# erhant/halo2-vectordb

Measured on AMD Instinct MI355X. Metric: constraints/sec, proving hot path (witness+layout+commit MSM+NTT), kmeans k=16 circuit, higher is better.
Workload: dtype u32x8 (BN254 Fr/Fq, 254-bit Montgomery)

## Files before the change

### halo2_vectordb_amd/csrc/limb9.hpp

```cpp
#pragma once
#include <math.h>

#include "field.hpp"

namespace vdb {

struct L9 {
  uint32_t l[9];
};
HD L9 l9_split(const u256& a) {
  L9 r;
#pragma unroll
  for (int k = 0; k < 9; k++) {
    int pb = 29 * k, wb = pb >> 5, ob = pb & 31;
    uint32_t lo = a.w[wb];
    uint32_t hi = wb + 1 < 8 ? a.w[wb + 1 < 8 ? wb + 1 : 0] : 0u;
    r.l[k] = ob ? ((lo >> ob) | (hi << (32 - ob))) : lo;
    if (k < 8) r.l[k] &= 0x1fffffffu;
  }
  return r;
}
HD L9 l9_split32(const u256& a) {
  L9 r;
  r.l[0] = (a.w[0] << 5) & 0x1fffffffu;
#pragma unroll
  for (int k = 1; k < 9; k++) {
    int pb = 29 * k - 5, wb = pb >> 5, ob = pb & 31;
    uint32_t lo = a.w[wb];
    uint32_t hi = wb + 1 < 8 ? a.w[wb + 1 < 8 ? wb + 1 : 0] : 0u;
    r.l[k] = ob ? ((lo >> ob) | (hi << (32 - ob))) : lo;
    if (k < 8) r.l[k] &= 0x1fffffffu;
  }
  return r;
}
HD u256 l9_pack(const L9& L) {
  u256 r;
  r.w[0] = L.l[0] | (L.l[1] << 29);
  r.w[1] = (L.l[1] >> 3) | (L.l[2] << 26);
  r.w[2] = (L.l[2] >> 6) | (L.l[3] << 23);
  r.w[3] = (L.l[3] >> 9) | (L.l[4] << 20);
  r.w[4] = (L.l[4] >> 12) | (L.l[5] << 17);
  r.w[5] = (L.l[5] >> 15) | (L.l[6] << 14);
  r.w[6] = (L.l[6] >> 18) | (L.l[7] << 11);
  r.w[7] = (L.l[7] >> 21) | (L.l[8] << 8);
  return r;
}
HD void l9_renorm(L9& x) {
  uint32_t c[8];
#pragma unroll
  for (int k = 0; k < 8; k++) c[k] = x.l[k] >> 29;
#pragma unroll
  for (int k = 0; k < 8; k++) x.l[k] &= 0x1fffffffu;
#pragma unroll
  for (int k = 1; k < 9; k++) x.l[k] += c[k - 1];
}
HD void l9_carry(L9& x) {
#pragma unroll
  for (int k = 0; k < 8; k++) {
    x.l[k + 1] += x.l[k] >> 29;
    x.l[k] &= 0x1fffffffu;
  }
}
HD L9 l9_add(const L9& a, const L9& b) {
  L9 r;
#pragma unroll
  for (int k = 0; k < 9; k++) r.l[k] = a.l[k] + b.l[k];
  return r;
}
HD L9 l9_sub(const L9& a, const L9& t, const uint32_t (&ckp)[9]) {
  L9 r;
#pragma unroll
  for (int k = 0; k < 9; k++) r.l[k] = a.l[k] + (ckp[k] - t.l[k]);
  return r;
}
HD L9 l9_neg(const L9& t, const uint32_t (&ckp)[9]) {
  L9 r;
#pragma unroll
  for (int k = 0; k < 9; k++) r.l[k] = ckp[k] - t.l[k];
  return r;
}
template <class M>
HD L9 l9_mul(const L9& a, const L9& b) {
  L9 r;
  mont_core29<M>(r.l, a.l, b.l);
  return r;
}
template <class M>
HD L9 l9_mul_shoup(const L9& v, const L9& w, const L9& wq) {
  L9 r;
  shoup_core29<M>(r.l, v.l, w.l, wq.l);
  return r;
}
template <class M>
HD L9 l9_mul2(const L9& a1, const L9& b1, const L9& a2, const L9& b2) {
  L9 r;
  mont_core29_2<M>(r.l, a1.l, b1.l, a2.l, b2.l);
  return r;
}
template <class M>
HD L9 l9_sqr(const L9& a) {
  L9 r;
  mont_sqr_core29<M>(r.l, a.l);
  return r;
}
template <class M>
HD u256 l9_canon(const L9& t) {
  return lazy_canon<M>(l9_pack(t));
}
template <class M>
HD bool l9_is_zero_mod(const L9& t) {
  uint32_t z = 0, e = 0;
#pragma unroll
  for (int k = 0; k < 9; k++) {
    z |= t.l[k];
    e |= t.l[k] ^ M::P29[k];
  }
  return z == 0 || e == 0;
}
template <class M>
inline double l9_offset_limbs(uint32_t K, uint32_t out[9]) {
  uint64_t carry = 0;
  for (int k = 0; k < 9; k++) {
    uint64_t v = (uint64_t)K * M::P29[k] + carry;
    out[k] = (uint32_t)(v & 0x1fffffffu);
    carry = v >> 29;
  }
  out[8] += (uint32_t)(carry << 29);
  out[0] += 1u << 29;
  for (int k = 1; k < 8; k++) out[k] += (1u << 29) - 1;
  out[8] -= 1;
  double cmax = 0;
  for (int k = 0; k < 8; k++) cmax = fmax(cmax, (double)out[k] / (double)(1u << 29));
  return cmax;
}

}
```

### halo2_vectordb_amd/csrc/ntt.hip

```cpp
#include <type_traits>
#include <vector>

#include "common.hpp"
#include "limb9.hpp"

namespace vdb {

#define NTT_THREADS 256
#define NTT_TILE 1024
#define NTT_MAX_PASSES 4
#define NTT_DEFAULT_COLGROUP 0x7fffffffu

struct NttPass {
  uint32_t log_n, S, log_inner, logG;
  uint32_t nprev;
  uint32_t prevS[NTT_MAX_PASSES];
  uint32_t first;
  uint32_t coset;
  uint32_t vslots;
  const u256* in_tab[4];
  uint32_t coset_out;
  uint32_t scale;
  uint32_t s0;
  uint64_t in_len;
  uint64_t in_stride, out_stride;
  uint32_t ren_mask;
  uint32_t ren_out;
  uint32_t blk0;
  const ColSrc* srcs;
  uint32_t n_blind;
  uint32_t n_cols;
  uint32_t col_group;
  u256 zeta1, zeta2, fin;
  u256 zeta0;
  uint32_t ckp[9];
  const uint32_t* sh_tab;
  uint32_t sh_res_log, sh_ns;
  int32_t sh_max_s;
};

__device__ __forceinline__ uint32_t bitrev_s(uint32_t x, uint32_t bits) { return bits ? (__brev(x) >> (32 - bits)) : 0u; }

__device__ __forceinline__ u256 l9_canon_wide(L9 x) {
  constexpr uint32_t MU = 2840127191u;
  const uint32_t q = __umulhi((x.l[8] + (x.l[7] >> 29)) << 3, MU) >> 24;
  uint64_t acc = 0;
#pragma unroll
  for (int k = 0; k < 9; k++) {
    const uint32_t nk = (k == 0 ? 0x20000000u : 0x1fffffffu) - FrParams::P29[k];
    acc += (uint64_t)x.l[k] + (uint64_t)q * nk;
    x.l[k] = (uint32_t)acc & 0x1fffffffu;
    acc >>= 29;
  }
  u256 v = l9_pack(x), t, p2, pp = mod_p<Fr>();
  u256_add(p2, pp, pp);
  uint32_t keep = u256_sub(t, v, p2);
#pragma unroll
  for (int i = 0; i < 8; i++) v.w[i] = keep ? v.w[i] : t.w[i];
  return lazy_canon<Fr>(v);
}
__device__ __forceinline__ L9 l9_mul(const L9& a, const L9& W) { return l9_mul<Fr>(a, W); }
__device__ __forceinline__ u256 l9_canon(const L9& t) { return l9_canon<Fr>(t); }

struct L9Planes {
  uint4* a;
  uint4* b;
  uint32_t* c;
};
__device__ __forceinline__ L9 lds_get(const L9Planes& P, uint32_t idx) {
  uint4 a = P.a[idx], b = P.b[idx];
  L9 r;
  r.l[0] = a.x; r.l[1] = a.y; r.l[2] = a.z; r.l[3] = a.w;
  r.l[4] = b.x; r.l[5] = b.y; r.l[6] = b.z; r.l[7] = b.w;
  r.l[8] = P.c[idx];
  return r;
}
__device__ __forceinline__ void lds_put(const L9Planes& P, uint32_t idx, const L9& v) {
  P.a[idx] = make_uint4(v.l[0], v.l[1], v.l[2], v.l[3]);
  P.b[idx] = make_uint4(v.l[4], v.l[5], v.l[6], v.l[7]);
  P.c[idx] = v.l[8];
}

template <uint32_t CS, uint32_t s, uint32_t step, class F>
__device__ __forceinline__ void ntt_static_steps(F&& f) {
  if constexpr (s < CS) {
    f(std::integral_constant<uint32_t, s>{}, std::integral_constant<uint32_t, step>{});
    ntt_static_steps<CS, (s + 1 < CS ? s + 2 : s + 1), step + 1>(f);
  }
}
constexpr uint32_t ntt_spec_sh_res_log(uint32_t cs) { return cs == 8 ? 0u : 2u; }
template <bool LAST, bool VS = false, uint32_t CS = 0, uint32_t CS0 = 0, uint32_t CREN = 0>
__global__ __launch_bounds__(NTT_THREADS) void k_ntt_pass(const u256* __restrict__ in, u256* __restrict__ out,
                                                         const u256* __restrict__ tw, const u256* __restrict__ tw_inter, NttPass p,
                                                         uint32_t tiles_per_col) {
  extern __shared__ uint4 smem[];
  constexpr bool SPEC = CS > 0;
  const uint32_t S = SPEC ? CS : p.S, P_logG = SPEC ? 10u - CS : p.logG, P_s0 = SPEC ? CS0 : p.s0, P_ren_mask = SPEC ? CREN : p.ren_mask;
  const uint32_t P_sh_res_log = SPEC ? ntt_spec_sh_res_log(CS) : p.sh_res_log, P_sh_ns = SPEC ? ((1u << (CS ? CS - 1 : 0)) >> ntt_spec_sh_res_log(CS)) : p.sh_ns;
  const int32_t P_sh_max_s = SPEC ? (int32_t)CS - 2 - (int32_t)ntt_spec_sh_res_log(CS) : p.sh_max_s;
  const bool P_shoup = SPEC ? true : p.sh_tab != nullptr, P_blk0 = SPEC ? true : p.blk0 != 0;
  const uint32_t m = 1u << S, G = 1u << P_logG, T = m * G;
  const uint32_t row = m + 1, NE = G * row, NW = m / 2 ? m / 2 : 1;
  L9Planes D, W;
  D.a = smem;
  D.b = D.a + NE;
  W.a = D.b + NE;
  W.b = W.a + NW;
  const uint32_t NS = P_shoup ? P_sh_ns : 0;
  L9Planes WS, WQ;
  WS.a = W.b + NW;
  WS.b = WS.a + NS;
  WQ.a = WS.b + NS;
  WQ.b = WQ.a + NS;
  D.c = reinterpret_cast<uint32_t*>(WQ.b + NS);
  W.c = D.c + NE;
  WS.c = W.c + NW;
  WQ.c = WS.c + NS;
  const uint32_t tid = threadIdx.x;
  uint32_t col, tile;
  if (p.col_group == 0) {
    col = blockIdx.x / tiles_per_col;
    tile = blockIdx.x % tiles_per_col;
  } else {
    const uint32_t per_group = p.col_group * tiles_per_col;
    const uint32_t grp = blockIdx.x / per_group, r = blockIdx.x % per_group;
    const uint32_t left = p.n_cols - grp * p.col_group, ncg = left < p.col_group ? left : p.col_group;
    col = grp * p.col_group + r % ncg;
    tile = r / ncg;
  }
  const u256* cin = in + (size_t)(VS ? col / p.vslots : col) * p.in_stride;
  const u256* ctab = nullptr;
  if constexpr (VS) {
    const uint32_t slot = col % p.vslots;
    ctab = slot == 0 ? p.in_tab[0] : (slot == 1 ? p.in_tab[1] : (slot == 2 ? p.in_tab[2] : p.in_tab[3]));
  }
  ColSrc csrc;
  const bool from_src = p.first && p.srcs != nullptr;
  if (from_src) csrc = p.srcs[col];
  u256* cout = out + (size_t)col * p.out_stride;

  uint64_t base;
  uint64_t jstride;
  uint64_t gstride;
  uint32_t i0 = 0, q0_base = 0, rdig = 0, rest = 1;
  if (!LAST) {
    uint32_t tiles_inner = (1u << p.log_inner) >> P_logG;
    uint32_t o = tile / tiles_inner;
    i0 = (tile % tiles_inner) << P_logG;
    base = ((uint64_t)o << (S + p.log_inner)) + i0;
    jstride = 1ull << p.log_inner;
    gstride = 1;
  } else {
    if (p.nprev == 0) {
      base = 0;
      jstride = 1;
      gstride = 0;
    } else {
      rest = 1u << (p.log_n - S - p.prevS[0]);
      q0_base = (tile / rest) << P_logG;
      rdig = tile % rest;
      base = ((uint64_t)q0_base * rest + rdig) << S;
      jstride = 1;
      gstride = (uint64_t)rest << S;
    }
  }

  for (uint32_t e = tid; e < m / 2; e += NTT_THREADS) lds_put(W, e, l9_split(ld256(tw + ((size_t)e << (p.log_n - S)))));
  for (uint32_t e = tid; e < NS; e += NTT_THREADS) {
    L9 ws, wq;
#pragma unroll
    for (int k = 0; k < 9; k++) {
      ws.l[k] = p.sh_tab[18 * e + k];
      wq.l[k] = p.sh_tab[18 * e + 9 + k];
    }
    lds_put(WS, e, ws);
    lds_put(WQ, e, wq);
  }
  const uint32_t mload = m >> P_s0, Tload = mload * G;
  L9 Z0, Z1, Z2;
  if (!VS && p.coset) {
    Z1 = l9_split(p.zeta1);
    Z2 = l9_split(p.zeta2);
    if (p.coset == 2) Z0 = l9_split(p.zeta0);
  }
  for (uint32_t e = tid; e < Tload; e += NTT_THREADS) {
    uint32_t j, g;
    if (!LAST) {
      g = e & (G - 1);
      j = e >> P_logG;
    } else {
      j = e & (mload - 1);
      g = e / mload;
    }
    uint64_t idx = base + j * jstride + g * gstride;
    L9 v;
    if (!p.first || idx < p.in_len) {
      v = l9_split(from_src ? colsrc_fetch(csrc, idx, 1ull << p.log_n, p.n_blind) : ld256(cin + idx));
      if constexpr (VS) {
        v = l9_mul(v, l9_split(ld256(ctab + idx)));
      } else if (p.coset) {
        uint32_t r3 = (uint32_t)(idx % 3);
        if (r3 == 1) v = l9_mul(v, Z1);
        else if (r3 == 2) v = l9_mul(v, Z2);
        else if (p.coset == 2) v = l9_mul(v, Z0);
      }
    } else {
#pragma unroll
      for (int k = 0; k < 9; k++) v.l[k] = 0;
    }
    for (uint32_t rep = 0; rep < (1u << P_s0); rep++) lds_put(D, g * row + j + rep * mload, v);
  }
  __syncthreads();
  auto do_step = [&](auto s_c, auto step_c) {
    const uint32_t s = s_c, step = step_c;
    const uint32_t logh = S - 1 - s, h = 1u << logh;
    const bool ren = (P_ren_mask >> step) & 1;
    if (s + 1 < S) {
      const uint32_t h2 = h >> 1, lh1 = logh ? logh - 1 : 0;
      auto radix4 = [&](auto first_c, auto ren_c, auto shoup_c, auto s2_c) {
        constexpr bool FIRST = decltype(first_c)::value, REN = decltype(ren_c)::value, SHOUP = decltype(shoup_c)::value, S2 = decltype(s2_c)::value;
        for (uint32_t t = tid; t < T / 4; t += NTT_THREADS) {
          uint32_t g, r, blk;
          if (S2) {
            const uint32_t lb = P_logG + lh1;
            blk = ((t >> lb) + blockIdx.x + (blockIdx.x >> 8)) & 3u;
            g = (t >> lh1) & (G - 1);
            r = t & (h2 - 1);
          } else {
            const uint32_t gi = t & ((m >> 2) - 1);
            g = t >> (S - 2);
            r = gi & (h2 - 1);
            blk = gi >> lh1;
          }
          const uint32_t j0 = g * row + (blk << (logh + 1)) + r;
          L9 x0 = lds_get(D, j0), x1 = lds_get(D, j0 + h2), x2 = lds_get(D, j0 + h), x3 = lds_get(D, j0 + h + h2);
          if (REN) {
            l9_renorm(x0);
            l9_renorm(x1);
            l9_renorm(x2);
            l9_renorm(x3);
          }
          if (FIRST) {
            L9 a0 = l9_add(x0, x2), a2 = l9_sub(x0, x2, p.ckp);
            L9 a1 = l9_add(x1, x3), a3 = l9_sub(x1, x3, p.ckp);
            l9_carry(a1);
            const L9 t3 = l9_mul(a3, lds_get(W, m >> 2));
            x0 = l9_add(a0, a1);
            x1 = l9_sub(a0, a1, p.ckp);
            x2 = l9_add(a2, t3);
            x3 = l9_sub(a2, t3, p.ckp);
          } else if (S2 && blk == 0) {
            l9_carry(x2);
            l9_carry(x3);
            L9 a0 = l9_add(x0, x2), a2 = l9_sub(x0, x2, p.ckp);
            L9 a1 = l9_add(x1, x3), a3 = l9_sub(x1, x3, p.ckp);
            l9_carry(a1);
            L9 t3;
            if (SHOUP) {
              const uint32_t iq = (m >> 2) >> P_sh_res_log;
              t3 = l9_mul_shoup<Fr>(a3, lds_get(WS, iq), lds_get(WQ, iq));
            } else {
              t3 = l9_mul(a3, lds_get(W, m >> 2));
            }
            x0 = l9_add(a0, a1);
            x1 = l9_sub(a0, a1, p.ckp);
            x2 = l9_add(a2, t3);
            x3 = l9_sub(a2, t3, p.ckp);
          } else if (SHOUP) {
            const uint32_t e = bitrev_s(blk, s) << logh, rl = P_sh_res_log;
            const uint32_t i0 = e >> rl, i1 = (e >> 1) >> rl, i2 = ((e >> 1) + (m >> 2)) >> rl;
            const L9 ws = lds_get(WS, i0), wq = lds_get(WQ, i0);
            const L9 t2 = l9_mul_shoup<Fr>(x2, ws, wq), t3 = l9_mul_shoup<Fr>(x3, ws, wq);
            const L9 a0 = l9_add(x0, t2), a2 = l9_sub(x0, t2, p.ckp);
            const L9 a1 = l9_add(x1, t3), a3 = l9_sub(x1, t3, p.ckp);
            const L9 u1 = l9_mul_shoup<Fr>(a1, lds_get(WS, i1), lds_get(WQ, i1));
            const L9 u3 = l9_mul_shoup<Fr>(a3, lds_get(WS, i2), lds_get(WQ, i2));
            x0 = l9_add(a0, u1);
            x1 = l9_sub(a0, u1, p.ckp);
            x2 = l9_add(a2, u3);
            x3 = l9_sub(a2, u3, p.ckp);
          } else {
            const uint32_t e = bitrev_s(blk, s) << logh;
            const L9 w = lds_get(W, e);
            const L9 t2 = l9_mul(x2, w), t3 = l9_mul(x3, w);
            const L9 a0 = l9_add(x0, t2), a2 = l9_sub(x0, t2, p.ckp);
            const L9 a1 = l9_add(x1, t3), a3 = l9_sub(x1, t3, p.ckp);
            const L9 u1 = l9_mul(a1, lds_get(W, e >> 1));
            const L9 u3 = l9_mul(a3, lds_get(W, (e >> 1) + (m >> 2)));
            x0 = l9_add(a0, u1);
            x1 = l9_sub(a0, u1, p.ckp);
            x2 = l9_add(a2, u3);
            x3 = l9_sub(a2, u3, p.ckp);
          }
          lds_put(D, j0, x0);
          lds_put(D, j0 + h2, x1);
          lds_put(D, j0 + h, x2);
          lds_put(D, j0 + h + h2, x3);
        }
      };
      using T_ = std::true_type;
      using F_ = std::false_type;
      const bool s2 = s == 2 && !ren && P_blk0;
      if (s == 0) {
        if (ren) radix4(T_{}, T_{}, F_{}, F_{});
        else radix4(T_{}, F_{}, F_{}, F_{});
      } else if (P_shoup && (int32_t)s <= P_sh_max_s) {
        if (ren) radix4(F_{}, T_{}, T_{}, F_{});
        else if (s2) radix4(F_{}, F_{}, T_{}, T_{});
        else radix4(F_{}, F_{}, T_{}, F_{});
      } else {
        if (ren) radix4(F_{}, T_{}, F_{}, F_{});
        else if (s2) radix4(F_{}, F_{}, F_{}, T_{});
        else radix4(F_{}, F_{}, F_{}, F_{});
      }
    } else {
      for (uint32_t b = tid; b < T / 2; b += NTT_THREADS) {
        const uint32_t g = b >> (S - 1), pj = b & ((m >> 1) - 1);
        const uint32_t r = pj & (h - 1), blk = pj >> logh, j0 = (blk << (logh + 1)) + r;
        const uint32_t a0 = g * row + j0, a1 = a0 + h;
        L9 u = lds_get(D, a0), v = lds_get(D, a1);
        if (ren) {
          l9_renorm(u);
          l9_renorm(v);
        }
        if (s) v = l9_mul(v, lds_get(W, bitrev_s(blk, s) << logh));
        lds_put(D, a0, l9_add(u, v));
        lds_put(D, a1, l9_sub(u, v, p.ckp));
      }
    }
    __syncthreads();
  };
  if constexpr (SPEC) {
    ntt_static_steps<CS, CS0, 0>(do_step);
  } else {
    uint32_t step = 0;
    for (uint32_t s = P_s0; s < S; step++) {
      do_step(s, step);
      s += (s + 1 < S) ? 2 : 1;
    }
  }
  L9 FIN, ZO1, ZO2;
  if (LAST && p.scale) FIN = l9_split(p.fin);
  if (LAST && p.coset_out) {
    ZO1 = l9_split(p.zeta2);
    ZO2 = l9_split(p.zeta1);
  }
  constexpr uint32_t EPT = NTT_TILE / NTT_THREADS;
  u256 twv[EPT];
  if (!LAST) {
#pragma unroll
    for (uint32_t it = 0; it < EPT; it++) {
      const uint32_t e = tid + it * NTT_THREADS;
      const uint32_t g = e & (G - 1), q = e >> P_logG;
      const uint64_t ex = ((uint64_t)q * ((uint64_t)i0 + g)) << (p.log_n - S - p.log_inner);
      if (e < T) twv[it] = ld256(tw_inter + ex);
    }
  }
#pragma unroll
  for (uint32_t it = 0; it < EPT; it++) {
    const uint32_t e = tid + it * NTT_THREADS;
    if (e >= T) break;
    uint32_t g = e & (G - 1), q = e >> P_logG;
    L9 v = lds_get(D, g * row + bitrev_s(q, S));
    if (p.ren_out) l9_renorm(v);
    if (!LAST) {
      v = l9_mul(v, l9_split(twv[it]));
      st256(cout + base + (uint64_t)q * jstride + g, l9_pack(v));
    } else {
      uint64_t pos;
      if (p.nprev == 0) {
        pos = q;
      } else {
        pos = (uint64_t)q0_base + g;
        uint32_t r = rdig;
        uint32_t shift = 0;
        for (uint32_t l = 0; l < p.nprev; l++) shift += p.prevS[l];
        for (int l = (int)p.nprev - 1; l >= 1; l--) {
          shift -= p.prevS[l];
          uint32_t ql = r & ((1u << p.prevS[l]) - 1);
          r >>= p.prevS[l];
          pos += (uint64_t)ql << shift;
        }
        pos += (uint64_t)q << (p.log_n - S);
      }
      if (p.scale) {
        v = l9_mul(v, FIN);
        const uint32_t r3 = p.coset_out ? (uint32_t)(pos % 3) : 0u;
        if (r3) v = l9_mul(v, r3 == 1 ? ZO1 : ZO2);
        st256(cout + pos, l9_canon(v));
      } else {
        const uint32_t r3 = p.coset_out ? (uint32_t)(pos % 3) : 0u;
        st256(cout + pos, r3 ? l9_canon(l9_mul(v, r3 == 1 ? ZO1 : ZO2)) : l9_canon_wide(v));
      }
    }
  }
}

__global__ __launch_bounds__(256) void k_twiddles(u256* __restrict__ tw, u256 omega, u256 m32, uint64_t n, uint32_t chunk) {
  uint64_t t = (uint64_t)blockIdx.x * blockDim.x + threadIdx.x;
  uint64_t lo = t * chunk;
  if (lo >= n) return;
  u256 w = mont_pow<Fr>(omega, u256_from_u64(lo));
  for (uint32_t i = 0; i < chunk && lo + i < n; i++) {
    st256(tw + lo + i, fr_mul(w, m32));
    w = fr_mul(w, omega);
  }
}

static const u256* get_twiddles(uint32_t log_n, const u256& omega, const u256& factor, bool scaled, int* err) {
  Context& c = ctx();
  Context::TwKey key{log_n | (scaled ? 0x80000000u : 0u), omega};
  auto it = c.twiddles.find(key);
  if (it != c.twiddles.end()) return it->second;
  uint64_t n = 1ull << log_n;
  u256* tw = nullptr;
  hipError_t e = hipMalloc(&tw, n * sizeof(u256));
  if (e != hipSuccess) {
    *err = hip_fail(e, "hipMalloc(twiddles)", __FILE__, __LINE__);
    return nullptr;
  }
  uint32_t chunk = 16;
  uint64_t threads = (n + chunk - 1) / chunk;
  {
    VDB_PROF("k_twiddles");
    hipLaunchKernelGGL(k_twiddles, dim3((unsigned)((threads + 255) / 256)), dim3(256), 0, c.stream, tw, omega, factor, n, chunk);
  }
  e = hipGetLastError();
  if (e != hipSuccess) {
    *err = hip_fail(e, "k_twiddles", __FILE__, __LINE__);
    (void)hipFree(tw);
    return nullptr;
  }
  c.twiddles[key] = tw;
  return tw;
}

static void limbs29(const u256& a, uint32_t extra_top , uint32_t out[9]) {
  for (int k = 0; k < 9; k++) {
    const int bit = 29 * k, wd = bit >> 5, sh = bit & 31;
    uint64_t v = wd < 8 ? (uint64_t)a.w[wd] >> sh : 0;
    if (sh && wd + 1 < 8) v |= (uint64_t)a.w[wd + 1] << (32 - sh);
    if (wd + 1 == 8 && sh) v |= (uint64_t)extra_top << (32 - sh);
    if (wd == 8) v = extra_top >> sh;
    out[k] = (uint32_t)v & 0x1fffffffu;
  }
}
static const uint32_t* get_shoup_table(uint32_t log_n, const u256& omega, uint32_t S, uint32_t res_log, int* err) {
  Context& c = ctx();
  Context::TwKey key{log_n | (S << 8) | (res_log << 16) | 0x40000000u, omega};
  auto it = c.twiddles.find(key);
  if (it != c.twiddles.end()) return reinterpret_cast<const uint32_t*>(it->second);
  const uint32_t m = 1u << S, ns = (m / 2) >> res_log;
  std::vector<uint32_t> tab((size_t)ns * 18);
  const u256 p = mod_p<Fr>();
  const u256 step = mont_pow<Fr>(omega, u256_from_u64(((uint64_t)1 << (log_n - S)) << res_log));
  u256 cur = mont_one<Fr>();
  for (uint32_t j = 0; j < ns; j++) {
    const u256 w = from_mont<Fr>(cur);
    limbs29(w, 0, &tab[18 * (size_t)j]);
    u256 r = w;
    uint32_t q[9] = {0, 0, 0, 0, 0, 0, 0, 0, 0};
    for (int b = 260; b >= 0; b--) {
      u256 d;
      u256_add(d, r, r);
      u256 t;
      const uint32_t borrow = u256_sub(t, d, p);
      r = borrow ? d : t;
      if (!borrow) q[b / 29] |= 1u << (b % 29);
    }
    for (int k = 0; k < 9; k++) tab[18 * (size_t)j + 9 + k] = q[k];
    cur = fr_mul(cur, step);
  }
  uint32_t* d = nullptr;
  hipError_t e = hipMalloc(&d, tab.size() * sizeof(uint32_t));
  if (e != hipSuccess) {
    *err = hip_fail(e, "hipMalloc(shoup table)", __FILE__, __LINE__);
    return nullptr;
  }
  e = hipMemcpy(d, tab.data(), tab.size() * sizeof(uint32_t), hipMemcpyHostToDevice);
  if (e != hipSuccess) {
    *err = hip_fail(e, "hipMemcpy(shoup table)", __FILE__, __LINE__);
    (void)hipFree(d);
    return nullptr;
  }
  c.twiddles[key] = reinterpret_cast<u256*>(d);
  return d;
}

int ntt_dev(u256* data, u256* out_or_null, size_t n_cols, uint32_t log_n, const u256& omega, bool scale_ninv,
            bool coset_in, size_t in_len, const ColSrc* srcs, uint32_t n_blind, bool coset_out, const u256* in_scale, const u256* const* in_tabs,
            uint32_t vslots) {
  Context& c = ctx();
  if (n_cols == 0) return VDB_OK;
  if (log_n > 26) {
    set_error("ntt: log_n > 26 unsupported");
    return VDB_ERR_ARG;
  }
  const uint64_t n = 1ull << log_n;
  const uint64_t in_stride = in_len ? in_len : n;
  if (!in_len) in_len = n;
  u256* dst = out_or_null ? out_or_null : data;
  if (!out_or_null && in_stride != n) {
    set_error("ntt: in-place transform needs in_len == n");
    return VDB_ERR_ARG;
  }
  if (vslots && (!out_or_null || !in_tabs || vslots > 4 || srcs || coset_in || n_cols % vslots)) {
    set_error("ntt: virtual columns need an output buffer and their input tables");
    return VDB_ERR_ARG;
  }
  if (srcs && (!out_or_null || in_len != n || log_n <= 10)) {
    set_error("ntt: column sources need an output buffer and a multi-pass size");
    return VDB_ERR_ARG;
  }
  int err = VDB_OK;
  const u256 m32 = host_fr_from_u64(32);
  const u256* tw = get_twiddles(log_n, omega, m32, false, &err);
  if (!tw) return err;

  uint32_t L, S[NTT_MAX_PASSES];
  if (log_n <= 10) {
    L = 1;
    S[0] = log_n;
  } else {
    static const uint32_t max_s = getenv("VDB_NTT_MAX_S") ? (uint32_t)atoi(getenv("VDB_NTT_MAX_S")) : 9u;
    uint32_t ms = max_s >= 4 && max_s <= 9 ? max_s : 9u;
    while ((log_n + ms - 1) / ms > NTT_MAX_PASSES) ms++;
    L = (log_n + ms - 1) / ms;
    for (uint32_t l = 0; l < L; l++) S[l] = log_n / L + (l < log_n % L ? 1 : 0);
  }
  const u256 fin = scale_ninv ? fr_mul(mont_inv<Fr>(host_fr_from_u64(n)), m32) : m32;
  const u256* tw_scaled = tw;
  if (scale_ninv && L > 1) {
    tw_scaled = get_twiddles(log_n, omega, fin, true, &err);
    if (!tw_scaled) return err;
  }
  u256 z1 = host_zeta(), z2 = fr_mul(z1, z1);
  z1 = fr_mul(z1, m32);
  z2 = fr_mul(z2, m32);
  u256 z0 = m32;
  if (in_scale) {
    z0 = fr_mul(z0, *in_scale);
    z1 = fr_mul(z1, *in_scale);
    z2 = fr_mul(z2, *in_scale);
  }
  static const bool shoup_on = !(getenv("VDB_NTT_SHOUP") && getenv("VDB_NTT_SHOUP")[0] == '0');
  uint32_t ckp[9];
  const double cmax = l9_offset_limbs<FrParams>(14, ckp);

  size_t chunk_cols = n_cols;
  u256* scratch = nullptr;
  if (L > 1) {
    size_t max_cols = ((size_t)2 << 30) / (n * sizeof(u256));
    if (max_cols < 1) max_cols = 1;
    if (chunk_cols > max_cols) chunk_cols = max_cols;
    if (vslots) chunk_cols = chunk_cols / vslots * vslots ? chunk_cols / vslots * vslots : vslots;
    scratch = (u256*)scratch_get(3, chunk_cols * n * sizeof(u256));
    if (!scratch) return VDB_ERR_OOM;
  }
  static const uint32_t col_group = getenv("VDB_NTT_COLGROUP") ? (uint32_t)strtoul(getenv("VDB_NTT_COLGROUP"), nullptr, 10) : NTT_DEFAULT_COLGROUP;
  for (size_t c0 = 0; c0 < n_cols; c0 += chunk_cols) {
    size_t nc = n_cols - c0 < chunk_cols ? n_cols - c0 : chunk_cols;
    uint32_t done_bits = 0;
    for (uint32_t l = 0; l < L; l++) {
      NttPass p;
      memset(&p, 0, sizeof(p));
      p.log_n = log_n;
      p.S = S[l];
      p.log_inner = log_n - done_bits - S[l];
      p.first = (l == 0);
      const bool last = (l == L - 1);
      p.coset = (l == 0 && coset_in) ? (in_scale ? 2u : 1u) : ((l == 0 && vslots) ? 3u : 0u);
      p.vslots = vslots;
      for (uint32_t t = 0; t < vslots; t++) p.in_tab[t] = in_tabs[t];
      p.zeta0 = z0;
      p.in_len = in_len;
      p.srcs = (l == 0 && srcs) ? srcs + c0 : nullptr;
      p.n_blind = n_blind;
      p.n_cols = (uint32_t)nc;
      p.col_group = last ? 0u : (col_group < nc ? col_group : (uint32_t)nc);
      p.zeta1 = z1;
      p.zeta2 = z2;
      p.fin = fin;
      memcpy(p.ckp, ckp, sizeof(ckp));
      p.scale = last && scale_ninv && L == 1;
      p.coset_out = last && coset_out;
      p.s0 = (l == 0 && !last && S[0] >= 3 && in_len * 4 <= n) ? 2 : 0;
      {
        double b = 1.0001;
        uint32_t step = 0;
        for (uint32_t st = p.s0; st < S[l]; step++) {
          if (st + 1 < S[l]) {
            if (st == 0) {
              b = 1.0 + 2.0 * cmax;
            } else {
              if (b + cmax >= 6.1 || b + 2.0 * cmax >= 7.95) {
                p.ren_mask |= 1u << step;
                b = 1.0001;
              }
              b += 2.0 * cmax;
            }
            st += 2;
          } else {
            if (st == 0) {
              b = 1.0 + cmax;
            } else {
              if (b >= 6.1 || b + cmax >= 7.95) {
                p.ren_mask |= 1u << step;
                b = 1.0001;
              }
              b += cmax;
            }
            st += 1;
          }
        }
        const bool out_mul = !last || p.scale || p.coset_out;
        static const bool blk0_on = !(getenv("VDB_NTT_BLK0") && getenv("VDB_NTT_BLK0")[0] == '0');
        p.blk0 = blk0_on ? 1u : 0u;
        static const bool always = getenv("VDB_NTT_REN_OUT") && getenv("VDB_NTT_REN_OUT")[0] == '1';
        p.ren_out = (always || (out_mul && b >= 6.1)) ? 1u : 0u;
      }
      const u256* src;
      u256* out;
      if (l == 0) {
        src = srcs ? scratch : data + (vslots ? c0 / vslots : c0) * in_stride;
        p.in_stride = in_stride;
      } else {
        src = scratch;
        p.in_stride = n;
      }
      if (last) {
        out = dst + c0 * n;
        p.out_stride = n;
      } else {
        out = scratch;
        p.out_stride = n;
      }
      uint32_t m = 1u << S[l];
      if (L == 1) {
        p.logG = 0;
        p.nprev = 0;
      } else {
        p.logG = 10 - S[l];
        const uint32_t room = last ? S[0] : p.log_inner;
        if (p.logG > room) p.logG = room;
        p.nprev = l;
        for (uint32_t q = 0; q < l && q < NTT_MAX_PASSES; q++) p.prevS[q] = S[q];
      }
      uint32_t G = 1u << p.logG;
      uint32_t tiles = (uint32_t)(n / ((uint64_t)m * G));
      size_t lds = (size_t)(G * (m + 1) + (m / 2 ? m / 2 : 1)) * (2 * sizeof(uint4) + sizeof(uint32_t));
      p.sh_tab = nullptr;
      p.sh_res_log = p.sh_ns = 0;
      p.sh_max_s = -1;
      if (shoup_on && S[l] >= 4) {
        const size_t room = (160 * 1024) / 3;
        uint32_t rl = 0;
        while (rl + 2 < S[l] && lds + (size_t)((m / 2) >> rl) * 72 > room) rl++;
        const int32_t max_s = (int32_t)S[l] - 2 - (int32_t)rl;
        if (lds + (size_t)((m / 2) >> rl) * 72 <= room && max_s >= 1) {
          p.sh_tab = get_shoup_table(log_n, omega, S[l], rl, &err);
          if (!p.sh_tab) return err;
          p.sh_res_log = rl;
          p.sh_ns = (m / 2) >> rl;
          p.sh_max_s = max_s;
          lds += (size_t)p.sh_ns * 72;
        }
      }
      dim3 grid((unsigned)(nc * tiles));
      if (lds > 64 * 1024) {
        bool& raised = c.ntt_lds_raised;
        if (!raised) {
          VDB_HIP(hipFuncSetAttribute((const void*)k_ntt_pass<true>, hipFuncAttributeMaxDynamicSharedMemorySize, 96 * 1024));
          VDB_HIP(hipFuncSetAttribute((const void*)k_ntt_pass<false>, hipFuncAttributeMaxDynamicSharedMemorySize, 96 * 1024));
          VDB_HIP(hipFuncSetAttribute((const void*)k_ntt_pass<true, true>, hipFuncAttributeMaxDynamicSharedMemorySize, 96 * 1024));
          VDB_HIP(hipFuncSetAttribute((const void*)k_ntt_pass<false, true>, hipFuncAttributeMaxDynamicSharedMemorySize, 96 * 1024));
          raised = true;
        }
      }
      static const bool spec_on = !(getenv("VDB_NTT_SPEC") && getenv("VDB_NTT_SPEC")[0] == '0');
      const u256* twi = last ? tw : (l == 0 ? tw_scaled : tw);
      const bool vs = (l == 0 && vslots);
      auto spec = [&](uint32_t cs, uint32_t cs0, uint32_t cren) {
        const uint32_t rl = ntt_spec_sh_res_log(cs);
        return spec_on && L > 1 && p.S == cs && p.s0 == cs0 && p.ren_mask == cren && p.logG == 10 - cs && p.sh_tab && p.blk0 && p.sh_res_log == rl &&
               p.sh_ns == ((1u << (cs - 1)) >> rl) && p.sh_max_s == (int32_t)cs - 2 - (int32_t)rl;
      };
#define NTT_LAUNCH(...) hipLaunchKernelGGL((k_ntt_pass<__VA_ARGS__>), grid, dim3(NTT_THREADS), lds, c.stream, src, out, tw, twi, p, tiles)
      {
        VDB_PROF("k_ntt_pass");
        if (last) {
          if (vs) NTT_LAUNCH(true, true);
          else if (spec(8, 0, 4)) NTT_LAUNCH(true, false, 8, 0, 4);
          else if (spec(9, 0, 20)) NTT_LAUNCH(true, false, 9, 0, 20);
          else NTT_LAUNCH(true, false);
        } else {
          if (vs && spec(8, 0, 4)) NTT_LAUNCH(false, true, 8, 0, 4);
          else if (vs) NTT_LAUNCH(false, true);
          else if (spec(8, 0, 4)) NTT_LAUNCH(false, false, 8, 0, 4);
          else if (spec(9, 2, 4)) NTT_LAUNCH(false, false, 9, 2, 4);
          else if (spec(9, 0, 20)) NTT_LAUNCH(false, false, 9, 0, 20);
          else NTT_LAUNCH(false, false);
        }
      }
#undef NTT_LAUNCH
      VDB_LAUNCH_CHECK();
      done_bits += S[l];
    }
  }
  return VDB_OK;
}

struct CosetMix {
  const u256* tab[4];
  u256 c[4][4];
};
__global__ __launch_bounds__(256) void k_cosets_combine(const u256* __restrict__ P, uint64_t n, uint32_t n_slots, CosetMix mx, u256* __restrict__ out) {
  const uint64_t i = (uint64_t)blockIdx.x * blockDim.x + threadIdx.x;
  if (i >= n) return;
  u256 v[4];
#pragma unroll
  for (uint32_t t = 0; t < 4; t++)
    if (t < n_slots) v[t] = fr_mul(ld256(P + t * n + i), ld256(mx.tab[t] + i));
#pragma unroll
  for (uint32_t j = 0; j < 4; j++) {
    if (j >= n_slots) break;
    u256 acc = fr_mul(v[0], mx.c[j][0]);
#pragma unroll
    for (uint32_t t = 1; t < 4; t++)
      if (t < n_slots) acc = fr_add(acc, fr_mul(v[t], mx.c[j][t]));
    st256(out + j * n + i, acc);
  }
}

u256 host_coset_shift(uint32_t k, uint32_t t) {
  static const uint32_t rev[4] = {0, 2, 1, 3};
  return fr_mul(host_zeta(), mont_pow<Fr>(host_root_of_unity(k + 2), u256_from_u64(rev[t & 3])));
}

static int host_cols_roundtrip(vdb_fr* const* cols, size_t n_cols, size_t n, u256** dbuf, bool upload) {
  Context& c = ctx();
  size_t bytes = n * sizeof(u256);
  if (upload) {
    *dbuf = (u256*)scratch_get(0, n_cols * bytes);
    if (!*dbuf) return VDB_ERR_OOM;
    for (size_t i = 0; i < n_cols; i++) VDB_HIP(hipMemcpyAsync(*dbuf + i * n, cols[i], bytes, hipMemcpyHostToDevice, c.stream));
  } else {
    for (size_t i = 0; i < n_cols; i++) VDB_HIP(hipMemcpyAsync(cols[i], *dbuf + i * n, bytes, hipMemcpyDeviceToHost, c.stream));
    VDB_HIP(hipStreamSynchronize(c.stream));
  }
  return VDB_OK;
}

}

using namespace vdb;

extern "C" {

int vdb_ntt_batch_dev(vdb_fr* cols_dev, size_t n_cols, uint32_t log_n, const vdb_fr* omega, int flags) {
  VDB_REQUIRE_INIT();
  VDB_ARG(cols_dev && omega, "null pointer");
  u256 w;
  memcpy(&w, omega, 32);
  return ntt_dev(as_u256(cols_dev), nullptr, n_cols, log_n, w, (flags & VDB_NTT_INVERSE_SCALE) != 0, false, 0, nullptr, 0, false, nullptr);
}
int vdb_ntt_batch(vdb_fr* const* cols, size_t n_cols, uint32_t log_n, const vdb_fr* omega, int flags) {
  VDB_REQUIRE_INIT();
  VDB_ARG(cols && omega, "null pointer");
  if (n_cols == 0) return VDB_OK;
  u256* d = nullptr;
  int rc = host_cols_roundtrip(cols, n_cols, (size_t)1 << log_n, &d, true);
  if (rc) return rc;
  rc = vdb_ntt_batch_dev(reinterpret_cast<vdb_fr*>(d), n_cols, log_n, omega, flags);
  if (rc) return rc;
  return host_cols_roundtrip(cols, n_cols, (size_t)1 << log_n, &d, false);
}
int vdb_lagrange_to_coeff_dev(vdb_fr* cols_dev, size_t n_cols, uint32_t k) {
  VDB_REQUIRE_INIT();
  VDB_ARG(cols_dev && k <= 26, "bad argument");
  u256 w = mont_inv<Fr>(host_root_of_unity(k));
  return ntt_dev(as_u256(cols_dev), nullptr, n_cols, k, w, true, false, 0, nullptr, 0, false, nullptr);
}
int vdb_lagrange_to_coeff_src_dev(const vdb_colsrc* src_dev, vdb_fr* coeff_dev, size_t n_cols, uint32_t k, uint32_t n_blind) {
  VDB_REQUIRE_INIT();
  VDB_ARG(src_dev && coeff_dev && k <= 26 && k > 10, "bad argument (column sources are supported for k > 10)");
  u256 w = mont_inv<Fr>(host_root_of_unity(k));
  return ntt_dev(nullptr, as_u256(coeff_dev), n_cols, k, w, true, false, 0, reinterpret_cast<const ColSrc*>(src_dev), n_blind, false, nullptr);
}
int vdb_lagrange_to_coeff(vdb_fr* const* cols, size_t n_cols, uint32_t k) {
  VDB_REQUIRE_INIT();
  VDB_ARG(cols, "null pointer");
  if (n_cols == 0) return VDB_OK;
  u256* d = nullptr;
  int rc = host_cols_roundtrip(cols, n_cols, (size_t)1 << k, &d, true);
  if (rc) return rc;
  rc = vdb_lagrange_to_coeff_dev(reinterpret_cast<vdb_fr*>(d), n_cols, k);
  if (rc) return rc;
  return host_cols_roundtrip(cols, n_cols, (size_t)1 << k, &d, false);
}
int vdb_coeff_to_extended_dev(const vdb_fr* coeff_dev, vdb_fr* ext_dev, size_t n_cols, uint32_t k, uint32_t ext_k) {
  VDB_REQUIRE_INIT();
  VDB_ARG(coeff_dev && ext_dev && k + ext_k <= 26, "bad argument");
  u256 w = host_root_of_unity(k + ext_k);
  return ntt_dev(const_cast<u256*>(as_u256(coeff_dev)), as_u256(ext_dev), n_cols, k + ext_k, w, false, true, (size_t)1 << k, nullptr, 0, false, nullptr);
}
int vdb_coeff_to_extended_scaled_dev(const vdb_fr* coeff_dev, vdb_fr* ext_dev, size_t n_cols, uint32_t k, uint32_t ext_k, const vdb_fr* scale) {
  VDB_REQUIRE_INIT();
  VDB_ARG(coeff_dev && ext_dev && scale && k + ext_k <= 26, "bad argument");
  u256 w = host_root_of_unity(k + ext_k), sv;
  memcpy(&sv, scale, 32);
  return ntt_dev(const_cast<u256*>(as_u256(coeff_dev)), as_u256(ext_dev), n_cols, k + ext_k, w, false, true, (size_t)1 << k, nullptr, 0, false, &sv);
}
int vdb_extended_to_coeff_dev(vdb_fr* ext_dev, size_t n_cols, uint32_t k, uint32_t ext_k) {
  VDB_REQUIRE_INIT();
  VDB_ARG(ext_dev && k + ext_k <= 26, "bad argument");
  u256 w = mont_inv<Fr>(host_root_of_unity(k + ext_k));
  return ntt_dev(as_u256(ext_dev), nullptr, n_cols, k + ext_k, w, true, false, 0, nullptr, 0, true, nullptr);
}
int vdb_coeff_to_cosets_dev(const vdb_fr* coeff_dev, vdb_fr* cosets_dev, size_t n_cols, uint32_t k, uint32_t n_slots, const vdb_fr* scale_or_null) {
  VDB_REQUIRE_INIT();
  VDB_ARG(coeff_dev && cosets_dev && k + 2 <= 26 && n_slots >= 1 && n_slots <= 4, "bad argument");
  if (n_cols == 0) return VDB_OK;
  Context& c = ctx();
  const uint64_t n = 1ull << k;
  const u256 m32 = host_fr_from_u64(32);
  const u256* tabs[4] = {nullptr, nullptr, nullptr, nullptr};
  int err = VDB_OK;
  if (scale_or_null) {
    u256 sv;
    memcpy(&sv, scale_or_null, 32);
    u256* buf = (u256*)scratch_get(6, (size_t)n_slots * n * sizeof(u256));
    if (!buf) return VDB_ERR_OOM;
    const uint32_t chunk = 16;
    const uint64_t threads = (n + chunk - 1) / chunk;
    for (uint32_t t = 0; t < n_slots; t++) {
      hipLaunchKernelGGL(k_twiddles, dim3((unsigned)((threads + 255) / 256)), dim3(256), 0, c.stream, buf + t * n, host_coset_shift(k, t), fr_mul(m32, sv), n, chunk);
      tabs[t] = buf + t * n;
    }
    VDB_LAUNCH_CHECK();
  } else {
    for (uint32_t t = 0; t < n_slots; t++) {
      tabs[t] = get_twiddles(k, host_coset_shift(k, t), m32, false, &err);
      if (!tabs[t]) return err;
    }
  }
  return ntt_dev(const_cast<u256*>(as_u256(coeff_dev)), as_u256(cosets_dev), n_cols * n_slots, k, host_root_of_unity(k), false, false, 0, nullptr, 0, false, nullptr,
                 tabs, n_slots);
}
int vdb_cosets_to_coeff_dev(vdb_fr* cosets_dev, vdb_fr* coeff_dev, uint32_t k, uint32_t n_slots) {
  VDB_REQUIRE_INIT();
  VDB_ARG(cosets_dev && coeff_dev && k + 2 <= 26 && n_slots >= 1 && n_slots <= 4, "bad argument");
  Context& c = ctx();
  const uint64_t n = 1ull << k;
// ... 56 lines not shown
```

Before: 1.892 billion.

## Use Shoup precomputed multipliers for all twiddle products in specialized NTT passes

In the specialized 256- and 512-point NTT kernels, every remaining Montgomery twiddle multiplication is replaced with a Shoup multiply. This covers the radix-4 inner constant, the radix-2 stage twiddle, the coset zeta scaling and the inter-pass twiddle. The shared-memory twiddle table is dropped, and device-side per-element Shoup records (value plus quotient, 80 bytes each) are built once and cached for the inter-pass multiply. The aim is cheaper field multiplies and less LDS use, paid for with more than double the global-memory bytes for inter-pass twiddle loads and extra cached table memory. Host-side Shoup table generation is factored into a shared header.

```diff
diff --git a/halo2_vectordb_amd/csrc/limb9.hpp b/halo2_vectordb_amd/csrc/limb9.hpp
--- a/halo2_vectordb_amd/csrc/limb9.hpp
+++ b/halo2_vectordb_amd/csrc/limb9.hpp
@@ -91,6 +91,32 @@
   shoup_core29<M>(r.l, v.l, w.l, wq.l);
   return r;
 }
+HD void limbs29(const u256& a, uint32_t out[9]) {
+#pragma unroll
+  for (int k = 0; k < 9; k++) {
+    const int bit = 29 * k, wd = bit >> 5, sh = bit & 31;
+    uint64_t v = (uint64_t)a.w[wd] >> sh;
+    if (sh && wd + 1 < 8) v |= (uint64_t)a.w[wd + 1 < 8 ? wd + 1 : 0] << (32 - sh);
+    out[k] = (uint32_t)v & 0x1fffffffu;
+  }
+}
+HD void shoup_pair29(const u256& w, uint32_t out[18]) {
+  limbs29(w, out);
+  const u256 p = mod_p<Fr>();
+  u256 r = w;
+#pragma unroll
+  for (int k = 8; k >= 0; k--) {
+    uint32_t d = 0;
+    for (int j = 28; j >= 0; j--) {
+      u256 s, t;
+      u256_add(s, r, r);
+      const uint32_t borrow = u256_sub(t, s, p);
+      r = borrow ? s : t;
+      d |= (borrow ^ 1u) << j;
+    }
+    out[9 + k] = d;
+  }
+}
 template <class M>
 HD L9 l9_mul2(const L9& a1, const L9& b1, const L9& a2, const L9& b2) {
   L9 r;
diff --git a/halo2_vectordb_amd/csrc/ntt.hip b/halo2_vectordb_amd/csrc/ntt.hip
--- a/halo2_vectordb_amd/csrc/ntt.hip
+++ b/halo2_vectordb_amd/csrc/ntt.hip
@@ -3,6 +3,7 @@
 
 #include "common.hpp"
 #include "limb9.hpp"
+#include "shoup_tables.hpp"
 
 namespace vdb {
 
@@ -37,9 +38,33 @@
   const uint32_t* sh_tab;
   uint32_t sh_res_log, sh_ns;
   int32_t sh_max_s;
+  const uint32_t* sh2_tab;
+  const uint4* tw_rec;
+  uint32_t zsh[3][18];
 };
 
 __device__ __forceinline__ uint32_t bitrev_s(uint32_t x, uint32_t bits) { return bits ? (__brev(x) >> (32 - bits)) : 0u; }
+__device__ __forceinline__ L9 kconst(const uint32_t* k) {
+  L9 r;
+#pragma unroll
+  for (int i = 0; i < 9; i++) r.l[i] = k[i];
+  return r;
+}
+__device__ __forceinline__ void ld_pair18(const uint32_t* e, L9& w, L9& wq) {
+  const uint2* q = reinterpret_cast<const uint2*>(e);
+  uint32_t t[18];
+#pragma unroll
+  for (int i = 0; i < 9; i++) {
+    const uint2 v = q[i];
+    t[2 * i] = v.x;
+    t[2 * i + 1] = v.y;
+  }
+#pragma unroll
+  for (int i = 0; i < 9; i++) {
+    w.l[i] = t[i];
+    wq.l[i] = t[9 + i];
+  }
+}
 
 __device__ __forceinline__ u256 l9_canon_wide(L9 x) {
   constexpr uint32_t MU = 2840127191u;
@@ -88,19 +113,20 @@
     ntt_static_steps<CS, (s + 1 < CS ? s + 2 : s + 1), step + 1>(f);
   }
 }
-constexpr uint32_t ntt_spec_sh_res_log(uint32_t cs) { return cs == 8 ? 0u : 2u; }
-template <bool LAST, bool VS = false, uint32_t CS = 0, uint32_t CS0 = 0, uint32_t CREN = 0>
+constexpr uint32_t ntt_spec_sh_res_log(uint32_t cs, bool sa) { return cs == 8 ? 0u : (sa ? 1u : 2u); }
+template <bool LAST, bool VS = false, uint32_t CS = 0, uint32_t CS0 = 0, uint32_t CREN = 0, bool SA = false>
 __global__ __launch_bounds__(NTT_THREADS) void k_ntt_pass(const u256* __restrict__ in, u256* __restrict__ out,
                                                          const u256* __restrict__ tw, const u256* __restrict__ tw_inter, NttPass p,
                                                          uint32_t tiles_per_col) {
   extern __shared__ uint4 smem[];
   constexpr bool SPEC = CS > 0;
+  static_assert(!SA || ((CS == 8 || CS == 9) && !VS), "SA: the 256- and 512-point instantiations, not the virtual-column one");
   const uint32_t S = SPEC ? CS : p.S, P_logG = SPEC ? 10u - CS : p.logG, P_s0 = SPEC ? CS0 : p.s0, P_ren_mask = SPEC ? CREN : p.ren_mask;
-  const uint32_t P_sh_res_log = SPEC ? ntt_spec_sh_res_log(CS) : p.sh_res_log, P_sh_ns = SPEC ? ((1u << (CS ? CS - 1 : 0)) >> ntt_spec_sh_res_log(CS)) : p.sh_ns;
-  const int32_t P_sh_max_s = SPEC ? (int32_t)CS - 2 - (int32_t)ntt_spec_sh_res_log(CS) : p.sh_max_s;
+  const uint32_t P_sh_res_log = SPEC ? ntt_spec_sh_res_log(CS, SA) : p.sh_res_log, P_sh_ns = SPEC ? ((1u << (CS ? CS - 1 : 0)) >> ntt_spec_sh_res_log(CS, SA)) : p.sh_ns;
+  const int32_t P_sh_max_s = SPEC ? (int32_t)CS - 2 - (int32_t)ntt_spec_sh_res_log(CS, SA) : p.sh_max_s;
   const bool P_shoup = SPEC ? true : p.sh_tab != nullptr, P_blk0 = SPEC ? true : p.blk0 != 0;
   const uint32_t m = 1u << S, G = 1u << P_logG, T = m * G;
-  const uint32_t row = m + 1, NE = G * row, NW = m / 2 ? m / 2 : 1;
+  const uint32_t row = m + 1, NE = G * row, NW = SA ? 0u : (m / 2 ? m / 2 : 1);
   L9Planes D, W;
   D.a = smem;
   D.b = D.a + NE;
@@ -165,7 +191,8 @@
     }
   }
 
-  for (uint32_t e = tid; e < m / 2; e += NTT_THREADS) lds_put(W, e, l9_split(ld256(tw + ((size_t)e << (p.log_n - S)))));
+  if (!SA)
+    for (uint32_t e = tid; e < m / 2; e += NTT_THREADS) lds_put(W, e, l9_split(ld256(tw + ((size_t)e << (p.log_n - S)))));
   for (uint32_t e = tid; e < NS; e += NTT_THREADS) {
     L9 ws, wq;
 #pragma unroll
@@ -198,6 +225,11 @@
       v = l9_split(from_src ? colsrc_fetch(csrc, idx, 1ull << p.log_n, p.n_blind) : ld256(cin + idx));
       if constexpr (VS) {
         v = l9_mul(v, l9_split(ld256(ctab + idx)));
+      } else if (SA && p.coset) {
+        const uint32_t r3 = (uint32_t)(idx % 3);
+        if (r3 == 1) v = l9_mul_shoup<Fr>(v, kconst(p.zsh[1]), kconst(p.zsh[1] + 9));
+        else if (r3 == 2) v = l9_mul_shoup<Fr>(v, kconst(p.zsh[2]), kconst(p.zsh[2] + 9));
+        else if (p.coset == 2) v = l9_mul_shoup<Fr>(v, kconst(p.zsh[0]), kconst(p.zsh[0] + 9));
       } else if (p.coset) {
         uint32_t r3 = (uint32_t)(idx % 3);
         if (r3 == 1) v = l9_mul(v, Z1);
@@ -211,10 +243,12 @@
     for (uint32_t rep = 0; rep < (1u << P_s0); rep++) lds_put(D, g * row + j + rep * mload, v);
   }
   __syncthreads();
+  L9 r2w, r2q;
   auto do_step = [&](auto s_c, auto step_c) {
     const uint32_t s = s_c, step = step_c;
     const uint32_t logh = S - 1 - s, h = 1u << logh;
     const bool ren = (P_ren_mask >> step) & 1;
+    if (SA && (S & 1) && s + 3 == S) ld_pair18(p.sh2_tab + 18 * bitrev_s(tid & ((m >> 1) - 1), S - 1), r2w, r2q);
     if (s + 1 < S) {
       const uint32_t h2 = h >> 1, lh1 = logh ? logh - 1 : 0;
       auto radix4 = [&](auto first_c, auto ren_c, auto shoup_c, auto s2_c) {
@@ -244,7 +278,13 @@
             L9 a0 = l9_add(x0, x2), a2 = l9_sub(x0, x2, p.ckp);
             L9 a1 = l9_add(x1, x3), a3 = l9_sub(x1, x3, p.ckp);
             l9_carry(a1);
-            const L9 t3 = l9_mul(a3, lds_get(W, m >> 2));
+            L9 t3;
+            if (SA) {
+              const uint32_t iq = (m >> 2) >> P_sh_res_log;
+              t3 = l9_mul_shoup<Fr>(a3, lds_get(WS, iq), lds_get(WQ, iq));
+            } else {
+              t3 = l9_mul(a3, lds_get(W, m >> 2));
+            }
             x0 = l9_add(a0, a1);
             x1 = l9_sub(a0, a1, p.ckp);
             x2 = l9_add(a2, t3);
@@ -323,7 +363,8 @@
           l9_renorm(u);
           l9_renorm(v);
         }
-        if (s) v = l9_mul(v, lds_get(W, bitrev_s(blk, s) << logh));
+        if (SA) v = l9_mul_shoup<Fr>(v, r2w, r2q);
+        else if (s) v = l9_mul(v, lds_get(W, bitrev_s(blk, s) << logh));
         lds_put(D, a0, l9_add(u, v));
         lds_put(D, a1, l9_sub(u, v, p.ckp));
       }
@@ -347,13 +388,23 @@
   }
   constexpr uint32_t EPT = NTT_TILE / NTT_THREADS;
   u256 twv[EPT];
+  L9 trw[SA ? EPT : 1], trq[SA ? EPT : 1];
   if (!LAST) {
 #pragma unroll
     for (uint32_t it = 0; it < EPT; it++) {
       const uint32_t e = tid + it * NTT_THREADS;
       const uint32_t g = e & (G - 1), q = e >> P_logG;
       const uint64_t ex = ((uint64_t)q * ((uint64_t)i0 + g)) << (p.log_n - S - p.log_inner);
-      if (e < T) twv[it] = ld256(tw_inter + ex);
+      if (e < T) {
+        if constexpr (SA) {
+          const uint4* rp = p.tw_rec + 5 * ex;
+          const uint4 r0 = rp[0], r1 = rp[1], r2 = rp[2], r3 = rp[3], r4 = rp[4];
+          trw[it] = L9{{r0.x, r0.y, r0.z, r0.w, r1.x, r1.y, r1.z, r1.w, r2.x}};
+          trq[it] = L9{{r2.y, r2.z, r2.w, r3.x, r3.y, r3.z, r3.w, r4.x, r4.y}};
+        } else {
+          twv[it] = ld256(tw_inter + ex);
+        }
+      }
     }
   }
 #pragma unroll
@@ -364,7 +415,8 @@
     L9 v = lds_get(D, g * row + bitrev_s(q, S));
     if (p.ren_out) l9_renorm(v);
     if (!LAST) {
-      v = l9_mul(v, l9_split(twv[it]));
+      if constexpr (SA) v = l9_mul_shoup<Fr>(v, trw[it], trq[it]);
+      else v = l9_mul(v, l9_split(twv[it]));
       st256(cout + base + (uint64_t)q * jstride + g, l9_pack(v));
     } else {
       uint64_t pos;
@@ -435,42 +487,12 @@
   return tw;
 }
 
-static void limbs29(const u256& a, uint32_t extra_top , uint32_t out[9]) {
-  for (int k = 0; k < 9; k++) {
-    const int bit = 29 * k, wd = bit >> 5, sh = bit & 31;
-    uint64_t v = wd < 8 ? (uint64_t)a.w[wd] >> sh : 0;
-    if (sh && wd + 1 < 8) v |= (uint64_t)a.w[wd + 1] << (32 - sh);
-    if (wd + 1 == 8 && sh) v |= (uint64_t)extra_top << (32 - sh);
-    if (wd == 8) v = extra_top >> sh;
-    out[k] = (uint32_t)v & 0x1fffffffu;
-  }
-}
 static const uint32_t* get_shoup_table(uint32_t log_n, const u256& omega, uint32_t S, uint32_t res_log, int* err) {
   Context& c = ctx();
   Context::TwKey key{log_n | (S << 8) | (res_log << 16) | 0x40000000u, omega};
   auto it = c.twiddles.find(key);
   if (it != c.twiddles.end()) return reinterpret_cast<const uint32_t*>(it->second);
-  const uint32_t m = 1u << S, ns = (m / 2) >> res_log;
-  std::vector<uint32_t> tab((size_t)ns * 18);
-  const u256 p = mod_p<Fr>();
-  const u256 step = mont_pow<Fr>(omega, u256_from_u64(((uint64_t)1 << (log_n - S)) << res_log));
-  u256 cur = mont_one<Fr>();
-  for (uint32_t j = 0; j < ns; j++) {
-    const u256 w = from_mont<Fr>(cur);
-    limbs29(w, 0, &tab[18 * (size_t)j]);
-    u256 r = w;
-    uint32_t q[9] = {0, 0, 0, 0, 0, 0, 0, 0, 0};
-    for (int b = 260; b >= 0; b--) {
-      u256 d;
-      u256_add(d, r, r);
-      u256 t;
-      const uint32_t borrow = u256_sub(t, d, p);
-      r = borrow ? d : t;
-      if (!borrow) q[b / 29] |= 1u << (b % 29);
-    }
-    for (int k = 0; k < 9; k++) tab[18 * (size_t)j + 9 + k] = q[k];
-    cur = fr_mul(cur, step);
-  }
+  const std::vector<uint32_t> tab = shoup_stage_entries(log_n, omega, S, res_log);
   uint32_t* d = nullptr;
   hipError_t e = hipMalloc(&d, tab.size() * sizeof(uint32_t));
   if (e != hipSuccess) {
@@ -480,6 +502,41 @@
   e = hipMemcpy(d, tab.data(), tab.size() * sizeof(uint32_t), hipMemcpyHostToDevice);
   if (e != hipSuccess) {
     *err = hip_fail(e, "hipMemcpy(shoup table)", __FILE__, __LINE__);
+    (void)hipFree(d);
+    return nullptr;
+  }
+  c.twiddles[key] = reinterpret_cast<u256*>(d);
+  return d;
+}
+
+__global__ __launch_bounds__(256) void k_shoup_records(const u256* __restrict__ tw, uint64_t n, u256 inv32, uint4* __restrict__ rec) {
+  const uint64_t e = (uint64_t)blockIdx.x * blockDim.x + threadIdx.x;
+  if (e >= n) return;
+  uint32_t o[20];
+  shoup_record_of_tw(ld256(tw + e), inv32, o);
+#pragma unroll
+  for (int i = 0; i < 5; i++) rec[5 * e + i] = make_uint4(o[4 * i], o[4 * i + 1], o[4 * i + 2], o[4 * i + 3]);
+}
+static const uint4* get_shoup_records(uint32_t log_n, const u256& omega, bool scaled, const u256* tw, int* err) {
+  Context& c = ctx();
+  Context::TwKey key{log_n | (scaled ? 0x80000000u : 0u) | 0x20000000u, omega};
+  auto it = c.twiddles.find(key);
+  if (it != c.twiddles.end()) return reinterpret_cast<const uint4*>(it->second);
+  const uint64_t n = 1ull << log_n;
+  uint4* d = nullptr;
+  hipError_t e = hipMalloc(&d, n * 5 * sizeof(uint4));
+  if (e != hipSuccess) {
+    *err = hip_fail(e, "hipMalloc(shoup records)", __FILE__, __LINE__);
+    return nullptr;
+  }
+  const u256 inv32 = mont_inv<Fr>(host_fr_from_u64(32));
+  {
+    VDB_PROF("k_shoup_records");
+    hipLaunchKernelGGL(k_shoup_records, dim3((unsigned)((n + 255) / 256)), dim3(256), 0, c.stream, tw, n, inv32, d);
+  }
+  e = hipGetLastError();
+  if (e != hipSuccess) {
+    *err = hip_fail(e, "k_shoup_records", __FILE__, __LINE__);
     (void)hipFree(d);
     return nullptr;
   }
@@ -538,10 +595,12 @@
   z1 = fr_mul(z1, m32);
   z2 = fr_mul(z2, m32);
   u256 z0 = m32;
+  u256 zc[3] = {mont_one<Fr>(), host_zeta(), fr_mul(host_zeta(), host_zeta())};
   if (in_scale) {
     z0 = fr_mul(z0, *in_scale);
     z1 = fr_mul(z1, *in_scale);
     z2 = fr_mul(z2, *in_scale);
+    for (int t = 0; t < 3; t++) zc[t] = fr_mul(zc[t], *in_scale);
   }
   static const bool shoup_on = !(getenv("VDB_NTT_SHOUP") && getenv("VDB_NTT_SHOUP")[0] == '0');
   uint32_t ckp[9];
@@ -648,7 +707,15 @@
       }
       uint32_t G = 1u << p.logG;
       uint32_t tiles = (uint32_t)(n / ((uint64_t)m * G));
-      size_t lds = (size_t)(G * (m + 1) + (m / 2 ? m / 2 : 1)) * (2 * sizeof(uint4) + sizeof(uint32_t));
+      static const bool spec_on = !(getenv("VDB_NTT_SPEC") && getenv("VDB_NTT_SPEC")[0] == '0');
+      const bool vs = (l == 0 && vslots);
+      auto spec_shape = [&](uint32_t cs, uint32_t cs0, uint32_t cren) {
+        return spec_on && L > 1 && p.S == cs && p.s0 == cs0 && p.ren_mask == cren && p.logG == 10 - cs && p.blk0;
+      };
+      static const bool shoup_all = !(getenv("VDB_NTT_SHOUP_ALL") && getenv("VDB_NTT_SHOUP_ALL")[0] == '0');
+      const bool sa = shoup_all && shoup_on && !vs && log_n <= 22 &&
+                      (spec_shape(8, 0, 4) || spec_shape(9, 0, 20) || (!last && spec_shape(9, 2, 4)));
+      size_t lds = (size_t)(G * (m + 1) + (sa ? 0 : (m / 2 ? m / 2 : 1))) * (2 * sizeof(uint4) + sizeof(uint32_t));
       p.sh_tab = nullptr;
       p.sh_res_log = p.sh_ns = 0;
       p.sh_max_s = -1;
@@ -677,28 +744,45 @@
           raised = true;
         }
       }
-      static const bool spec_on = !(getenv("VDB_NTT_SPEC") && getenv("VDB_NTT_SPEC")[0] == '0');
       const u256* twi = last ? tw : (l == 0 ? tw_scaled : tw);
-      const bool vs = (l == 0 && vslots);
-      auto spec = [&](uint32_t cs, uint32_t cs0, uint32_t cren) {
-        const uint32_t rl = ntt_spec_sh_res_log(cs);
-        return spec_on && L > 1 && p.S == cs && p.s0 == cs0 && p.ren_mask == cren && p.logG == 10 - cs && p.sh_tab && p.blk0 && p.sh_res_log == rl &&
-               p.sh_ns == ((1u << (cs - 1)) >> rl) && p.sh_max_s == (int32_t)cs - 2 - (int32_t)rl;
+      auto spec = [&](uint32_t cs, uint32_t cs0, uint32_t cren, bool sa_) {
+        const uint32_t rl = ntt_spec_sh_res_log(cs, sa_);
+        return spec_shape(cs, cs0, cren) && p.sh_tab && p.sh_res_log == rl && p.sh_ns == ((1u << (cs - 1)) >> rl) && p.sh_max_s == (int32_t)cs - 2 - (int32_t)rl;
       };
+      if (sa) {
+        if (!spec(p.S, p.s0, p.ren_mask, true)) {
+          set_error("ntt: SA plan does not match its instantiation");
+          return VDB_ERR_ARG;
+        }
+        if (S[l] & 1) {
+          p.sh2_tab = get_shoup_table(log_n, omega, S[l], 0, &err);
+          if (!p.sh2_tab) return err;
+        }
+        if (!last) {
+          p.tw_rec = get_shoup_records(log_n, omega, twi != tw, twi, &err);
+          if (!p.tw_rec) return err;
+        }
+        for (int t = 0; t < 3; t++) shoup_const_of_mont(zc[t], p.zsh[t]);
+      }
 #define NTT_LAUNCH(...) hipLaunchKernelGGL((k_ntt_pass<__VA_ARGS__>), grid, dim3(NTT_THREADS), lds, c.stream, src, out, tw, twi, p, tiles)
       {
         VDB_PROF("k_ntt_pass");
         if (last) {
           if (vs) NTT_LAUNCH(true, true);
-          else if (spec(8, 0, 4)) NTT_LAUNCH(true, false, 8, 0, 4);
-          else if (spec(9, 0, 20)) NTT_LAUNCH(true, false, 9, 0, 20);
+          else if (sa && p.S == 8) NTT_LAUNCH(true, false, 8, 0, 4, true);
+          else if (sa) NTT_LAUNCH(true, false, 9, 0, 20, true);
+          else if (spec(8, 0, 4, false)) NTT_LAUNCH(true, false, 8, 0, 4);
+          else if (spec(9, 0, 20, false)) NTT_LAUNCH(true, false, 9, 0, 20);
           else NTT_LAUNCH(true, false);
         } else {
-          if (vs && spec(8, 0, 4)) NTT_LAUNCH(false, true, 8, 0, 4);
+          if (vs && spec(8, 0, 4, false)) NTT_LAUNCH(false, true, 8, 0, 4);
           else if (vs) NTT_LAUNCH(false, true);
-          else if (spec(8, 0, 4)) NTT_LAUNCH(false, false, 8, 0, 4);
-          else if (spec(9, 2, 4)) NTT_LAUNCH(false, false, 9, 2, 4);
-          else if (spec(9, 0, 20)) NTT_LAUNCH(false, false, 9, 0, 20);
+          else if (sa && p.S == 8) NTT_LAUNCH(false, false, 8, 0, 4, true);
+          else if (sa && p.s0 == 2) NTT_LAUNCH(false, false, 9, 2, 4, true);
+          else if (sa) NTT_LAUNCH(false, false, 9, 0, 20, true);
+          else if (spec(8, 0, 4, false)) NTT_LAUNCH(false, false, 8, 0, 4);
+          else if (spec(9, 2, 4, false)) NTT_LAUNCH(false, false, 9, 2, 4);
+          else if (spec(9, 0, 20, false)) NTT_LAUNCH(false, false, 9, 0, 20);
           else NTT_LAUNCH(false, false);
         }
       }
diff --git a/halo2_vectordb_amd/csrc/shoup_tables.hpp b/halo2_vectordb_amd/csrc/shoup_tables.hpp
--- /dev/null
+++ b/halo2_vectordb_amd/csrc/shoup_tables.hpp
@@ -0,0 +1,27 @@
+#pragma once
+#include <vector>
+
+#include "limb9.hpp"
+
+namespace vdb {
+
+inline void shoup_const_of_mont(const u256& mont, uint32_t out[18]) { shoup_pair29(from_mont<Fr>(mont), out); }
+
+inline std::vector<uint32_t> shoup_stage_entries(uint32_t log_n, const u256& omega, uint32_t S, uint32_t res_log) {
+  const uint32_t m = 1u << S, ns = (m / 2) >> res_log;
+  std::vector<uint32_t> tab((size_t)ns * 18);
+  const u256 step = mont_pow<Fr>(omega, u256_from_u64(((uint64_t)1 << (log_n - S)) << res_log));
+  u256 cur = mont_one<Fr>();
+  for (uint32_t j = 0; j < ns; j++) {
+    shoup_const_of_mont(cur, &tab[18 * (size_t)j]);
+    cur = fr_mul(cur, step);
+  }
+  return tab;
+}
+
+HD void shoup_record_of_tw(const u256& t, const u256& inv32, uint32_t out[20]) {
+  shoup_pair29(from_mont<Fr>(fr_mul(t, inv32)), out);
+  out[18] = out[19] = 0;
+}
+
+}
```

Result: faster. 1.944 billion, median of 6 (+2.7%).
